# gvanhoy/gr-liquiddsp

Hardware: AMD Instinct MI355X
Metric: Msamples/s through flex_rx (QPSK r1/2 1024B) (higher is better)
Workload: dtype f32; 1 GPU; flex_rx single stream per GPU, 20000000 samples (10 Msym), PSK4 r=1/2 (CONV_V27), 1024-B payload, CRC-24, 256-sample gaps, CFO/phase/delay + AWGN Es/N0=20 dB; frames_decoded_ok=1154, streams_per_gpu=1, blocks_in_flight=12, stage_events=none (fxrx_set_timing level 0), steps=1415, passes=independent captures (reset between passes), segments=256, repairs=0

## Files before the change

### gr-liquiddsp_amd/csrc/fx_host.cpp

```cpp
#include <hip/hip_runtime.h>
#include <algorithm>
#include <chrono>
#include <cmath>
#include <cstdio>
#include <cstdlib>
#include <cstring>
#include <memory>
#include <string>
#include <vector>
#include "../../include/fxrx.h"
#include "fx_device.h"
#include "fx_codec.hpp"
#include "fx_launch.h"
#include "fx_traffic.h"

namespace {

thread_local std::string g_err;
void set_err(const std::string &s) { g_err = s; }

#define HIP_OK(expr)                                                                          \
    do {                                                                                      \
        hipError_t e_ = (expr);                                                               \
        if (e_ != hipSuccess) {                                                               \
// ... 648 lines not shown
    if (!detect && c->cfg.soft_decision && (sl.d_soft.reserve(8 * sl.byte_cap) || (c->cfg.want_framesyms && sl.h_soft.reserve(8 * sl.byte_cap)))) return FXRX_ERR_HIP;
#ifdef FX_STAMPS
    if (!detect && sl.d_pres.reserve(chain_slots)) return FXRX_ERR_HIP;
#endif
    std::memcpy(sl.hp_desc.p, jobs.data(), NJ * sizeof(FxWalkJob));
    uint32_t *hl = reinterpret_cast<uint32_t *>(sl.hp_desc.p + o_list);
    if (!early.empty()) std::memcpy(hl, early.data(), early.size() * sizeof(uint32_t));
    if (!late.empty()) std::memcpy(hl + early.size(), late.data(), late.size() * sizeof(uint32_t));
    if (!spec.empty()) std::memcpy(hl + NJ, spec.data(), spec.size() * sizeof(uint32_t));
    std::memcpy(sl.hp_desc.p + o_streams, sds.data(), NS * sizeof(FxStreamDesc));
    const uint32_t *d_list = sl.job_list();

    const double tp2 = g_prof_on ? prof_now() : 0.0;
    if (!sl.ingest.empty()) {
        std::vector<IngestJob> todo; todo.swap(sl.ingest);
        const size_t bytes = iq_sample_bytes(sl.ingest_fmt);
        for (const IngestJob &j : todo) {
            const void *src = j.dev_src;
            if (!src) { HIP_OK(hipMemcpyAsync(sl.d_raw[j.stream].p, j.host_src, j.n * bytes, hipMemcpyHostToDevice, st)); src = sl.d_raw[j.stream].p; }
            HIP_OK(fx_launch_ingest(st, sl.ingest_fmt, src, sl.d_in[j.stream].p, (size_t)j.n, sl.ingest_scale, (unsigned)c->n_cus));
        }
    }
    HIP_OK(fx_launch_upload(st, sl.hp_desc.p, sl.d_desc.p, desc_bytes, (unsigned)c->n_cus));
    const int tl = c->timing_level >= 0 ? c->timing_level : (c->depth > 1 ? 0 : 2);
    sl.timing_level = tl;
    if (c->debug_walk_twice > 0) HIP_OK(fx_launch_prescan(st, (unsigned)spec.size(), sl.ps_words, sl.jobs(), d_list + NJ, c->d_tables));
    for (int rep = 0; rep < c->debug_walk_twice; rep++) HIP_OK(launch_walk(c, sl, st, d_list, (unsigned)early.size()));
    if (tl >= 2) HIP_OK(hipEventRecord(sl.ev[kEvStart], st));
    if (c->debug_walk_twice <= 0) HIP_OK(fx_launch_prescan(st, (unsigned)spec.size(), sl.ps_words, sl.jobs(), d_list + NJ, c->d_tables));
    HIP_OK(launch_walk(c, sl, st, d_list, (unsigned)early.size()));
    const bool verify = !detect && c->skip_seek && !sl.force_noskip;
    hipStream_t cst = st;
    if (!late.empty()) {
        if (verify) {
            HIP_OK(fx_launch_copy_u32(st, &sl.hdr_walk()->n_runs, &sl.hdr_walk()->runs_done));
            HIP_OK(launch_seekverify(c, sl, st, c->verify_per_cu * (unsigned)c->n_cus, 0u));
        }
        if (!c->st_chain) {
            int lo = 0, hi = 0;
            HIP_OK(hipDeviceGetStreamPriorityRange(&lo, &hi));
            HIP_OK(hipStreamCreateWithPriority(&c->st_chain, hipStreamNonBlocking, hi));
        }
        HIP_OK(hipEventRecord(sl.ev[kEvHandover], st));
        cst = c->st_chain;
        HIP_OK(hipStreamWaitEvent(cst, sl.ev[kEvHandover], 0));
        if (c->prev_chain) HIP_OK(hipStreamWaitEvent(cst, c->prev_chain, 0));
        HIP_OK(launch_walk(c, sl, cst, d_list + early.size(), (unsigned)late.size()));
    }
    if (tl >= 2) HIP_OK(hipEventRecord(sl.ev[kEvWalk], cst));
    if (verify)
        HIP_OK(launch_seekverify(c, sl, cst, late.empty() ? c->verify_per_cu * (unsigned)c->n_cus : (unsigned)std::min<size_t>((size_t)c->verify_per_cu * (size_t)c->n_cus, std::max<size_t>(64, 16 * late.size())), 1u));
    if (tl >= 2) HIP_OK(hipEventRecord(sl.ev[kEvVerify], cst));
    if (late.empty() && c->prev_chain) HIP_OK(hipStreamWaitEvent(cst, c->prev_chain, 0));
    if (c->carry_reader[(b + 1) % 3]) HIP_OK(hipStreamWaitEvent(cst, c->carry_reader[(b + 1) % 3], 0));
    const double tp3 = g_prof_on ? prof_now() : 0.0;
    const int rb = enqueue_back(c, sl, kChainFast, cst, may_defer);
    if (g_prof_on) { const double tp4 = prof_now(); g_prof[1] += tp1 - tp0; g_prof[2] += tp2 - tp1; g_prof[3] += tp3 - tp2; g_prof[4] += tp4 - tp3; g_prof_n++; }
    return rb;
}

static FxVbpreMember vbpre_member(Slot &sl, uint32_t first_wave, uint32_t n_waves)
{
    return FxVbpreMember{ sl.d_pjobs.p, sl.dec_list(kDecBatch), sl.hdr_pay(), sl.d_hard.p, sl.d_bufA.p, sl.d_bufB.p, sl.h_out.p, sl.h_recs.p, sl.h_hdr.p, first_wave, n_waves };
}
static int launch_tails(fxrx_ctx_s *c, Slot *const *m, unsigned n)
{
    hipStream_t st = m[n - 1]->st;
    for (unsigned i = 0; i + 1 < n; i++) HIP_OK(hipStreamWaitEvent(st, m[i]->ev[kEvMf], 0));
    auto done = [&]() -> int {
        for (unsigned i = 0; i < n; i++) { HIP_OK(hipEventRecord(m[i]->ev[kEvDone], st)); m[i]->tail_launched = true; m[i]->tail_st = st; }
        if (n > 1) { c->gang_launches++; c->gang_members += n; }
        return 0;
    };
    {
        FxPllGang g; unsigned waves[FX_GANG_MAX]; g.n = n;
        for (unsigned i = 0; i < n; i++) { const Slot &sl = *m[i]; g.m[i] = FxPllMember{ sl.d_pjobs.p, sl.d_pll_list.p, sl.hdr_pay(), sl.d_symraw.p, sl.d_symraw.p, sl.d_hard.p, sl.h_recs.p }; waves[i] = sl.tail.pll_waves; }
        HIP_OK(fx_launch_paypll(&g, waves, c->pll_waves, st, c->d_tables));
    }
    for (unsigned i = 0; i < n; i++) if (m[i]->timing_level >= 1) HIP_OK(hipEventRecord(m[i]->ev[kEvPll], st));
    if (c->debug_stop_after == 6) return done();
    for (unsigned i = 0; i < n; i++) {
        Slot &sl = *m[i];
        if (c->cfg.soft_decision) {
            HIP_OK(fx_launch_softdemod(sl.tail.mf_grid, st, sl.d_pjobs.p, sl.d_mf_job.p, sl.d_mf_c0.p, sl.hdr_pay(), sl.d_symraw.p, sl.d_hard.p, sl.d_soft.p, c->d_tables));
            if (c->cfg.want_framesyms) HIP_OK(hipMemcpyAsync(sl.h_soft.p, sl.d_soft.p, 8 * sl.byte_cap, hipMemcpyDeviceToHost, st));
        }
        HIP_OK(launch_decoders(c, sl, st, 0u, sl.tail.plain, sl.tail.rs));
    }
    {
        FxVbpreGang g; g.n = n;
        for (unsigned i = 0; i < n; i++) g.m[i] = vbpre_member(*m[i], 0u, m[i]->vb_blk ? m[i]->tail.vb_pre : 0u);
        HIP_OK(fx_launch_vbpre(&g, st, c->d_tables, c->vb_clean ? 1 : 0, c->vb_early_tail && c->vb_clean ? 1 : 0));
    }
    for (unsigned i = 0; i < n; i++) {
        Slot &sl = *m[i];
        if (sl.vb_blk) HIP_OK(launch_trellis(c, sl, st, sl.tail.vb_items, sl.tail.vb_packed, sl.tail.with_fix, sl.tail.vb_fin, sl.tail.fb));
        if (sl.timing_level >= 2) HIP_OK(hipEventRecord(sl.ev[kEvDec], st));
        if (c->cfg.want_framesyms) HIP_OK(fx_launch_symcopy(2u * (unsigned)c->n_cus, st, sl.hdr_pay(), sl.d_symraw.p, sl.h_framesyms.p));
    }
    return done();
}

static int close_gang(fxrx_ctx_s *c)
{
    if (c->gang.empty()) return 0;
    if (c->gang.size() > FX_GANG_MAX) { set_err("open gang larger than FX_GANG_MAX (internal error)"); return FXRX_ERR_STATE; }
    Slot *m[FX_GANG_MAX]; unsigned n = 0;
    for (Slot *s : c->gang) m[n++] = s;
    c->gang.clear();
    return launch_tails(c, m, n);
}

static int enqueue_back(fxrx_ctx_s *c, Slot &sl, int chain_mode, hipStream_t chain_st, bool may_defer)
{
    const unsigned NS = c->cfg.n_streams; const bool detect = c->cfg.mode == FXRX_MODE_DETECTOR;
    const uint64_t b = sl.seq; const uint32_t chain_slots = sl.chain_cap; hipStream_t st = sl.st;
    sl.tail_launched = true; sl.tail_st = st;
    if (chain_mode == kChainFull)
        HIP_OK(fx_launch_chain(detect ? FX_MODE_DETECT : FX_MODE_FLEXRX, c->cfg.equalizer ? 1 : 0, c->cfg.soft_header ? 1 : 0, NS, st, sl.streams(), sl.jobs(), (uint32_t)sl.NJ, sl.d_wres.p, sl.d_frames.p, sl.d_chain.p,
                               sl.d_chain_count.p, sl.d_runs.p, sl.run_cap, sl.hdr_walk(), c->chain_slow ? 1u : 0u, c->d_tables));
    else if (chain_mode == kChainFast) {
        hipStream_t cs = chain_st ? chain_st : st;
        sl.inchain = !c->chain_slow && (c->inchain_repair == 2 || (c->inchain_repair == 1 && c->inchain_left > 0));
        if (c->inchain_left) c->inchain_left--;
        if (!sl.inchain) HIP_OK(launch_chainfast(c, sl, cs, kStitch));
        else {
            HIP_OK(launch_chainfast(c, sl, cs, kStitchPass1));
            HIP_OK(launch_walk(c, sl, cs, sl.d_req.p, (unsigned)std::min<size_t>(2 * sl.NJ, 64), kWalkRequestsInChain));
            HIP_OK(launch_chainfast(c, sl, cs, kStitchPass2));
        }
    }
    HIP_OK(hipEventRecord(sl.ev[kEvChain], chain_mode == kChainFast && chain_st ? chain_st : st));
    if (chain_mode == kChainFast && chain_st && chain_st != st) HIP_OK(hipStreamWaitEvent(st, sl.ev[kEvChain], 0));
    c->prev_chain = sl.ev[kEvChain];
    {
        FxPlanArgs a;
        a.streams = sl.streams(); a.nstreams = NS; a.detect = detect ? 1u : 0u; a.eq = c->cfg.equalizer ? 1u : 0u; a.vb_blk = sl.vb_blk;
        a.chain = sl.d_chain.p; a.chain_count = sl.d_chain_count.p; a.stream_base = sl.d_stream_base.p;
        a.pjobs = sl.d_pjobs.p; a.recs = sl.h_recs.p;
        a.mf_job = sl.d_mf_job.p; a.mf_c0 = sl.d_mf_c0.p; a.mf_cap = sl.mf_cap;
        a.pll_list = sl.d_pll_list.p; a.dec_list = sl.dec_list(kDecPlain); a.list_cap = sl.list_cap();
        a.vb_items = sl.d_vb_items.p; a.vb_cap = sl.vb_cap;
        a.hdr = sl.hdr_walk(); a.hdr_pay = sl.hdr_pay(); a.hdr_host = sl.h_hdr.p; a.ws = sl.d_plan_ws.p;
        HIP_OK(fx_launch_plan(st, c->plan_grid ? c->plan_grid : (unsigned)std::min<uint64_t>(64, c->traffic.frames / 2048 + 1), c->plan_fused ? 1 : 0, c->plan_threads, a));
    }
    const int tl = sl.timing_level;
    if (tl >= 2) HIP_OK(hipEventRecord(sl.ev[kEvPlan], st));
    if (c->debug_stop_after == 4) { c->carry_reader[b % 3] = nullptr; HIP_OK(hipEventRecord(sl.ev[kEvDone], st)); return 0; }
    if (!detect) {
        const TailPlan plan = plan_tail(c->traffic, TailCaps{ chain_slots, sl.mf_cap, sl.vb_cap, sl.vb_blk }, TailKnobs{ c->depth, c->n_cus, c->mf_per_cu, c->vb_debug, c->vb_early_tail, c->vb_clean });
        HIP_OK(fx_launch_paymf(plan.mf_grid, c->cfg.equalizer ? 1 : 0, st, sl.d_pjobs.p, sl.d_mf_job.p, sl.d_mf_c0.p, sl.hdr_pay(), sl.d_chain.p, sl.d_symraw.p, c->d_tables));
        HIP_OK(hipEventRecord(sl.ev[kEvMf], st));
        c->carry_reader[b % 3] = sl.ev[kEvMf];
        if (c->debug_stop_after == 5) { HIP_OK(hipEventRecord(sl.ev[kEvDone], st)); return 0; }
        sl.tail = plan;
        if (sl.vb_blk && c->traffic.trellis_left) c->traffic.trellis_left--;
        sl.timing.trellis_launched = plan.vb_fin ? 1 : 0;
        unsigned ahead = 0;
        for (unsigned k = 0; k < c->inflight; k++) ahead += c->slots[(c->tail + k) % (c->depth + 1)]->tail_launched ? 1u : 0u;
        const unsigned G = c->tail_gang;
        if (G >= 2 && may_defer && c->depth >= 4 && c->traffic.seen && !c->debug_stop_after && tl <= 1 && ahead >= G) {
            sl.tail_launched = false; sl.tail_st = nullptr;
            c->gang.push_back(&sl);
            return c->gang.size() >= G ? close_gang(c) : 0;
        }
        { const int r = close_gang(c); if (r) return r; }
        Slot *one = &sl;
        return launch_tails(c, &one, 1u);
    } else {
        if (c->cfg.want_framesyms) HIP_OK(launch_detwin(c, sl, 0u, sl.win_reserved, false));
        HIP_OK(hipEventRecord(sl.ev[kEvMf], st));
        if (tl >= 1) HIP_OK(hipEventRecord(sl.ev[kEvPll], st));
        if (tl >= 2) HIP_OK(hipEventRecord(sl.ev[kEvDec], st));
        c->carry_reader[b % 3] = sl.ev[kEvMf];
    }
    HIP_OK(hipEventRecord(sl.ev[kEvDone], st));
    return 0;
}

static int prepare_ingest(fxrx_ctx_s *c, Slot &sl, const void *const *iq, const uint64_t *n_samples, int on_device, int fmt)
{
    const unsigned NS = c->cfg.n_streams;
    const size_t bytes = iq_sample_bytes(fmt);
    sl.ingest.clear();
    for (unsigned s = 0; s < NS; s++)
        if (n_samples[s] && (!iq[s] || (reinterpret_cast<uintptr_t>(iq[s]) & (bytes - 1)))) {
            set_err("fxrx_submit_fmt: integer IQ must be aligned to its sample size (sc16: 4 bytes, sc8: 2 bytes)"); return FXRX_ERR_ARG;
        }
    if (sl.d_in.size() < NS) sl.d_in.resize(NS);
    if (sl.d_raw.size() < NS) sl.d_raw.resize(NS);
    std::vector<IngestJob> jobs;
    for (unsigned s = 0; s < NS; s++) {
        const uint64_t nn = n_samples[s];
        if (sl.d_in[s].reserve(nn + 1)) return FXRX_ERR_HIP;
        if (!nn) continue;
        IngestJob j; j.stream = s; j.n = nn;
        if (on_device) j.dev_src = iq[s];
        else if (!(nn * bytes <= c->ingest_kernel_max && pinned_device_ptr(iq[s], &j.dev_src, 0u))) {
            j.dev_src = nullptr; j.host_src = iq[s];
            if (sl.d_raw[s].reserve(nn * bytes + 16)) return FXRX_ERR_HIP;
        }
        jobs.push_back(j);
    }
    sl.ingest.swap(jobs); sl.ingest_fmt = fmt; sl.ingest_scale = c->iq_scale[fmt];
    return 0;
}

static int submit_block(fxrx_ctx *c, const void *const *iq, const uint64_t *n_samples, int on_device, int fmt)
{
    if (!c || !iq || !n_samples) { set_err("fxrx_submit: null argument"); return FXRX_ERR_ARG; }
    if (iq_sample_bytes(fmt) == 0) { set_err("fxrx_submit_fmt: unknown IQ format"); return FXRX_ERR_ARG; }
    if (c->inflight >= c->depth) { set_err("fxrx_submit: pipeline full, call fxrx_collect first"); return FXRX_ERR_STATE; }
    HIP_OK(hipSetDevice(c->cfg.device));
    const auto t_enter = std::chrono::steady_clock::now();
    const unsigned NS = c->cfg.n_streams;
    const unsigned nslots = c->depth + 1;
    Slot &sl = *c->slots[c->head];
    sl.ingest.clear();
    if (fmt != FXRX_IQ_FC32) { const int r = prepare_ingest(c, sl, iq, n_samples, on_device, fmt); if (r) return r; }
    sl.out.clear(); sl.timing = fxrx_timing{};
    sl.kept_hops = sl.kept_cheap = sl.kept_vhops = sl.kept_vfail = sl.kept_repairs = 0;
    const unsigned noskip_before = c->noskip_left;
    sl.force_noskip = c->noskip_left > 0; if (c->noskip_left) c->noskip_left--;
    sl.seq = c->seq;
    sl.x.assign(NS, nullptr); sl.n.assign(n_samples, n_samples + NS); sl.snap.assign(NS, StreamSnap{});
    if (sl.d_in.size() < NS) sl.d_in.resize(NS);
    struct Undo { fxrx_ctx_s *c; std::vector<StreamState> st; unsigned noskip; bool armed = true;
                  ~Undo() { if (armed) { c->st = st; c->noskip_left = noskip; } } } undo{ c, c->st, noskip_before };
    uint64_t total_new = 0;
    for (unsigned s = 0; s < NS; s++) {
        StreamState &S = c->st[s];
        const uint64_t nn = n_samples[s];
        total_new += nn;
        if (fmt != FXRX_IQ_FC32) sl.x[s] = sl.d_in[s].p;
// ... 513 lines not shown
```

### gr-liquiddsp_amd/csrc/fx_kernels.hip

```cpp
#include <hip/hip_runtime.h>
#include <algorithm>
#include "fx_device.h"
#include "fx_launch.h"
#include "fx_vbclean.h"
#include "fx_rsgmd.h"

#define HALF         256

template <int WW> struct WalkLdsT {
    static constexpr int WAVES = WW;
    static constexpr bool SWEEP_PAIRS = WW == 4;
    float2 win[FX_NFFT];
    float2 X[FX_NFFT];
    float2 S[FX_NFFT];
    float2 scr[WW][576];
    float2 v[640];
    float2 P[256];
    float  m2[FX_NFFT];
    float2 hdr[FX_HDR_SYM];
    float2 cw[(WW + 1) * FX_HOP + 8];
    __device__ __forceinline__ float2 *scr2(int wave) { return wave < 2 ? v + 576 * wave : cw + 576 * (wave - 2); }
    float2 pb[16];
    float2 eqw[16];
    float  taps[FX_MF_TAPS];
// ... 2177 lines not shown
                const uint32_t g = t0 + k, sub = tid & 15u;
                for (uint32_t b = sub; b < kp.y; b += 16u) if (kp.x + b < a.vb_cap) { a.vb_items[kp.x + b] = g; a.vb_items[a.vb_cap + kp.x + b] = b; }
                for (uint32_t c = sub; c < kp.w; c += 16u) if (kp.z + c < a.mf_cap) { a.mf_job[kp.z + c] = g; a.mf_c0[kp.z + c] = c * 1024u; }
            }
            __syncthreads();
        }
    }
    plan_pad_lists<NT>(cnt, sh.cls_base, sh.vbc_base, a);
    PLAN_TICK(st6_);
    __threadfence(); __syncthreads();
    PLAN_TICK(st7_);
    if (tid == 0) {
#ifdef FX_STAMPS
        sh.h.stamp[1] = st1_; sh.h.stamp[2] = st2_; sh.h.stamp[6] = st6_; sh.h.stamp[7] = st7_;
#endif
        plan_fill_hdr(sh.h, N, run, cnt, sh.cls_base, sh.vbc_base, a);
    }
    __syncthreads();
    plan_mirror_hdr<NT>(sh.h, a);
}

extern "C" hipError_t fx_launch_plan(hipStream_t st, unsigned grid, int fused, unsigned threads, const FxPlanArgs &a)
{
    const unsigned g = grid < 1u ? 1u : (grid > PLAN_MAXG ? PLAN_MAXG : grid);
    if (fused && g == 1u) {
        if (threads == 512u) hipLaunchKernelGGL((fx_planfused_kernel<512>), dim3(1), dim3(512), 0, st, a);
        else if (threads == 256u) hipLaunchKernelGGL((fx_planfused_kernel<256>), dim3(1), dim3(256), 0, st, a);
        else return hipErrorInvalidValue;
    } else {
        hipLaunchKernelGGL(fx_plan_kernel, dim3(g), dim3(PLAN_THREADS), 0, st, a);
        hipLaunchKernelGGL(fx_planlists_kernel, dim3(g), dim3(PLAN_THREADS), 0, st, a);
    }
    return hipGetLastError();
}
extern "C" unsigned fx_plan_ws_words(void) { return PW_WORDS; }

#define PMF_THREADS 256
#define PMF_SYMS    1024
#define PMF_SPAN    (2 * PMF_SYMS + FX_MF_TAPS)

__global__ __launch_bounds__(PMF_THREADS)
void fx_paymf_kernel(const FxPayJob *jobs, const uint32_t *blk_job, const uint32_t *blk_c0, const FxBlockHdr *hdr, const FxFrame *chain, float2 *sym_raw,
                     const FxTables *T)
{
    constexpr int LEAD = FX_EQ_TAPS - 1;
    __shared__ float2 v[PMF_SPAN + LEAD + 4];
    __shared__ float2 u[2 * PMF_SYMS + FX_EQ_TAPS];
    __shared__ float2 eqw[16];
    __shared__ float taps[FX_MF_TAPS];
    const uint32_t nitems = hdr->n_mfblk;
    const int tid = threadIdx.x;
    const float2 *sc = T->sc;
    for (uint32_t bi = blockIdx.x; bi < nitems; bi += gridDim.x) {
        const FxPayJob job = jobs[blk_job[bi]];
        const uint32_t c0 = blk_c0[bi];
        const uint32_t ns = min((uint32_t)PMF_SYMS, job.nsym - c0);
        const int64_t sym0 = (int64_t)FX_SYM0_PAY + FX_EQ_DELAY;
        const int64_t nlo = sym_sample(sym0 + c0, job.mfc0) - LEAD - (FX_MF_TAPS - 1);
        const int64_t nhi = sym_sample(sym0 + c0 + ns - 1, job.mfc0);
        const int span = (int)(nhi - nlo + 1);
        const XSrc xs = make_xsrc(job.x, job.xa_end, 0);
        __syncthreads();
        if (tid < FX_MF_TAPS) taps[tid] = T->proto[job.pfb + FX_NPFB * tid];
        if (tid < 16) eqw[tid] = tid < FX_EQ_TAPS ? chain[job.chain_idx].eq[tid] : make_float2(0.0f, 0.0f);
        for (int m = tid; m < span; m += PMF_THREADS) {
            const int64_t nn = nlo + m;
            v[m] = derot(xld(xs, job.start + nn), job.mix_th + job.mix_dl * (uint32_t)nn, sc);
        }
        __syncthreads();
        const int nu = span - (FX_MF_TAPS - 1);
        for (int m = tid; m < nu; m += PMF_THREADS) {
            const float2 y = mf_sum<7>(v, taps, m + (FX_MF_TAPS - 1));
            u[m] = make_float2(y.x * job.mf_scale, y.y * job.mf_scale);
        }
        __syncthreads();
        for (uint32_t i = tid; i < ns; i += PMF_THREADS) {
            const int nc = (int)(sym_sample(sym0 + c0 + i, job.mfc0) - nlo) - (FX_MF_TAPS - 1);
            sym_raw[(size_t)job.sym_off + c0 + i] = eq_sum16(u + nc - (FX_EQ_TAPS - 1), eqw);
        }
    }
}

#define PMF4_STRIDE 274
extern "C" __global__ __launch_bounds__(PMF_THREADS)
void fx_paymf4_kernel(const FxPayJob *jobs, const uint32_t *blk_job, const uint32_t *blk_c0, const FxBlockHdr *hdr, float2 *sym_raw, const FxTables *T)
{
    __shared__ float2 ph[8 * PMF4_STRIDE];
    __shared__ __attribute__((aligned(16))) float taps[FX_MF_TAPS];
    static_assert(FX_MF_TAPS == 28 && PMF_SYMS == 4 * PMF_THREADS, "tile below: 28 taps, four symbols per thread");
    static_assert(PMF4_STRIDE >= (PMF_SPAN + 8) / 8 + 5, "phase arrays hold the span plus the slack phantom symbols read");
    const uint32_t nitems = hdr->n_mfblk;
    const int tid = threadIdx.x;
    const float2 *sc = T->sc;
    for (uint32_t bi = blockIdx.x; bi < nitems; bi += gridDim.x) {
        const FxPayJob job = jobs[blk_job[bi]];
        const uint32_t c0 = blk_c0[bi];
        const uint32_t ns = min((uint32_t)PMF_SYMS, job.nsym - c0);
        const int64_t nlo = sym_sample((int64_t)FX_SYM0_PAY + c0, job.mfc0) - (FX_MF_TAPS - 1);
        const int span = 2 * (int)ns + (FX_MF_TAPS - 2);
        const float2 *px = job.x, *pa = job.xa_end;
        const int64_t p0 = job.start + nlo;
        const uint32_t th0 = job.mix_th + job.mix_dl * (uint32_t)nlo, dl = job.mix_dl;
        __syncthreads();
        if (tid < FX_MF_TAPS) taps[tid] = T->proto[job.pfb + FX_NPFB * tid];
        constexpr int NLD = (PMF_SPAN + PMF_THREADS - 1) / PMF_THREADS;
        float2 raw[NLD];
#pragma unroll
        for (int k = 0; k < NLD; k++) {
            const int m = tid + PMF_THREADS * k;
            const int64_t p = p0 + m;
            raw[k] = m < span ? (p < 0 ? pa[p] : px[p]) : make_float2(0.0f, 0.0f);
        }
#pragma unroll
        for (int k = 0; k < NLD; k++) {
            const int m = tid + PMF_THREADS * k;
            const int j = m >> 1;
            if (m < span) ph[((m & 1) * 4 + (j & 3)) * PMF4_STRIDE + (j >> 2)] = derot(raw[k], th0 + dl * (uint32_t)m, sc);
        }
        __syncthreads();
        if (4u * (uint32_t)tid < ns) {
            float2 e[17], o[17];
#pragma unroll
            for (int j = 0; j < 17; j++) {
                e[j] = ph[(j & 3) * PMF4_STRIDE + tid + (j >> 2)];
                o[j] = ph[(4 + (j & 3)) * PMF4_STRIDE + tid + (j >> 2)];
            }
            float h[FX_MF_TAPS];
#pragma unroll
            for (int q = 0; q < FX_MF_TAPS / 4; q++) { const float4 t4 = reinterpret_cast<const float4 *>(taps)[q]; h[4 * q] = t4.x; h[4 * q + 1] = t4.y; h[4 * q + 2] = t4.z; h[4 * q + 3] = t4.w; }
            float yr[4], yi[4];
#pragma unroll
            for (int r = 0; r < 4; r++) {
                float ar = 0.0f, ai = 0.0f;
#pragma unroll
                for (int k = 0; k < 14; k++) {
                    ar = fmaf(h[2 * k], o[13 + r - k].x, ar); ai = fmaf(h[2 * k], o[13 + r - k].y, ai);
                    ar = fmaf(h[2 * k + 1], e[13 + r - k].x, ar); ai = fmaf(h[2 * k + 1], e[13 + r - k].y, ai);
                }
                yr[r] = ar * job.mf_scale; yi[r] = ai * job.mf_scale;
            }
            float4 *dst = reinterpret_cast<float4 *>(sym_raw + (size_t)job.sym_off + c0 + 4u * (uint32_t)tid);
            dst[0] = make_float4(yr[0], yi[0], yr[1], yi[1]);
            dst[1] = make_float4(yr[2], yi[2], yr[3], yi[3]);
        }
    }
}

extern "C" hipError_t fx_launch_paymf(unsigned grid, int eq, hipStream_t st, const FxPayJob *jobs, const uint32_t *blk_job, const uint32_t *blk_c0, const FxBlockHdr *hdr,
                                      const FxFrame *chain, float2 *sym_raw, const FxTables *T)
{
    if (grid == 0) return hipSuccess;
    if (eq) hipLaunchKernelGGL(fx_paymf_kernel, dim3(grid), dim3(PMF_THREADS), 0, st, jobs, blk_job, blk_c0, hdr, chain, sym_raw, T);
    else hipLaunchKernelGGL(fx_paymf4_kernel, dim3(grid), dim3(PMF_THREADS), 0, st, jobs, blk_job, blk_c0, hdr, sym_raw, T);
    return hipGetLastError();
}

#define PLL_THREADS 64
#define PLL_MAX_WAVES 4
#define PLL_BLK     8

__device__ __forceinline__ void pll_load8(const float4 *p, float4 b[4]) { b[0] = p[0]; b[1] = p[1]; b[2] = p[2]; b[3] = p[3]; }

template <int MS>
__device__ __forceinline__ unsigned pll_demod(float2 r, unsigned &prev, const float2 *sc, float2 &xh, float &pe)
{
    if constexpr (MS == FX_MODEM_PSK2 || MS == FX_MODEM_PSK4) {
        unsigned idx; float pr, pim;
        if constexpr (MS == FX_MODEM_PSK2) {
            const bool neg = !(r.x > 0.0f);
            idx = neg ? 1u : 0u;
            xh = make_float2(neg ? -1.0f : 1.0f, 0.0f);
            pr = neg ? -r.x : r.x; pim = neg ? -r.y : r.y;
        } else {
            const bool horiz = fabsf(r.x) >= fabsf(r.y);
            const bool neg = horiz ? !(r.x > 0.0f) : !(r.y > 0.0f);
            idx = (horiz ? 0u : 1u) + (neg ? 2u : 0u);
            const float sg = neg ? -1.0f : 1.0f;
            xh = horiz ? make_float2(sg, 0.0f) : make_float2(0.0f, sg);
            const float a = horiz ? r.x : r.y, b = horiz ? r.y : -r.x;
            pr = neg ? -a : a; pim = neg ? -b : b;
        }
        (void)pr;
        pe = pim;
        return gray_enc(idx);
    } else {
        return modem_demod((unsigned)MS, modem_bps((unsigned)MS), r, prev, sc, xh, pe);
    }
}

template <int MS, bool TAIL>
__device__ __forceinline__ void pll_block8(const float4 (&cur)[4], unsigned live, uint32_t &th, float &fq, float &evm, unsigned &prev, const float2 *sc,
                                           float4 *out, uint2 *hd)
{
    float rr[2 * PLL_BLK]; unsigned h0 = 0, h1 = 0;
    float wc, ws; sincos_u32(th, sc, wc, ws);
#pragma unroll
    for (int k = 0; k < PLL_BLK; k++) {
        const float4 v4 = cur[k >> 1];
        const float2 y = (k & 1) ? make_float2(v4.z, v4.w) : make_float2(v4.x, v4.y);
        float2 r = make_float2(fmaf(y.x, wc, y.y * ws), fmaf(y.y, wc, -(y.x * ws))), xh; float pe;
        unsigned pv = prev;
        const unsigned s = pll_demod<MS>(r, pv, sc, xh, pe);
        if (!TAIL || (unsigned)k < live) {
            float dr = r.x - xh.x, di = r.y - xh.y;
            evm += fmaf(dr, dr, di * di);
            fq = fmaf(pe, 68356.5248f, fq);
            const float t = phase_step(fmaf(pe, 6835652.5f, fq));
            th += (uint32_t)(int)t;
            float cd, sd; sincos_small(t, cd, sd);
            const float c2 = fmaf(wc, cd, -(ws * sd)), s2 = fmaf(ws, cd, wc * sd);
            wc = c2; ws = s2;
            prev = pv;
        }
        rr[2 * k] = r.x; rr[2 * k + 1] = r.y;
        if (k < 4) h0 |= s << (8 * k); else h1 |= s << (8 * (k - 4));
    }
#pragma unroll
    for (int k = 0; k < 4; k++) out[k] = make_float4(rr[4 * k], rr[4 * k + 1], rr[4 * k + 2], rr[4 * k + 3]);
    *hd = make_uint2(h0, h1);
}

template <int MS>
__device__ __forceinline__ void pll_frame(uint32_t f, const FxPayJob *jobs, const float2 *sc, const float2 *sym_raw, float2 *framesyms, uint8_t *hard, FxOutRec *recs)
{
    if (f == 0xFFFFFFFFu) return;
    const FxPayJob job = jobs[f];
    const float4 *in = reinterpret_cast<const float4 *>(sym_raw + job.sym_off);
// ... 2165 lines not shown
```

### gr-liquiddsp_amd/csrc/fx_traffic.h

```cpp
#pragma once
#include <algorithm>
#include <stdint.h>
#include "fx_common.h"

constexpr unsigned kTrellisHold = 8;
constexpr uint32_t kFallbackWaves = 32;

struct Traffic {
    bool seen = false;
    uint64_t samples = 0, frames = 0;
    uint64_t plain = 0, rs = 0;
    uint64_t batch = 0, vb_items = 0;
    uint64_t vb_steps = 0;
    uint64_t vb_fix = 0;
    uint64_t fb = 0;
    uint64_t mf_items = 0;
    uint32_t verify_per = 4;
    unsigned trellis_left = 0;

    void observe(const FxBlockHdr &h, uint64_t vb_rep, uint64_t vb_clean, bool vb_early, uint64_t n_samples, int n_cus)
    {
        samples = n_samples; frames = h.n_frames; plain = h.n_dec_plain; batch = h.n_dec_batch; vb_items = h.n_vb_items; mf_items = h.n_mfblk;
        vb_steps = (uint64_t)h.vb_want * (h.vb_blk ? h.vb_blk : 1u);
        fb = h.n_vb_fallback; vb_fix = h.n_vb_fallback + vb_rep;
        if (vb_early && h.n_dec_batch > vb_clean) trellis_left = kTrellisHold;
        rs = h.n_dec_rs ? h.n_dec_rs : rs - std::min<uint64_t>(rs, std::max<uint64_t>(1, rs / 8));
        if (h.verify_hops) verify_per = (uint32_t)std::min<uint64_t>(16, std::max<uint64_t>(1, ((uint64_t)h.verify_hops + 4ull * n_cus - 1) / (4ull * n_cus)));
        seen = true;
    }
};

inline uint32_t with_margin(uint64_t count, uint64_t cap, uint64_t extra = 64, uint64_t floor = 0) { return (uint32_t)std::min(cap, std::max(floor, count + count / 2 + extra)); }

struct TailPlan {
    uint32_t pll_waves = 0, mf_grid = 0;
    uint32_t plain = 0, rs = 0;
    uint32_t vb_pre = 0, vb_items = 0, vb_fin = 0, fb = 0;
    int vb_packed = 0, with_fix = 0;
    bool vb_early = false;
};
struct TailCaps { uint32_t chain_slots, mf_cap, vb_cap, vb_blk; };
struct TailKnobs { unsigned depth; int n_cus; uint32_t mf_per_cu, vb_debug; bool vb_early_tail, vb_clean; };

inline TailPlan plan_tail(const Traffic &t, const TailCaps &cap, const TailKnobs &k)
{
    const uint64_t slots = cap.chain_slots, cus = (uint64_t)k.n_cus;
    TailPlan p;
    p.pll_waves = (t.frames ? with_margin(t.frames, slots) : cap.chain_slots) / 64 + FX_PLL_CLASSES;
    p.mf_grid = (uint32_t)std::min<uint64_t>(cap.mf_cap, k.mf_per_cu ? k.mf_per_cu * cus : std::max<uint64_t>(8 * cus, t.mf_items + t.mf_items / 8 + 64));
    p.vb_early = cap.vb_blk && k.vb_early_tail && k.vb_clean;
    const bool trellis = cap.vb_blk && (!p.vb_early || !t.seen || k.vb_debug || t.trellis_left > 0);
    if (!t.seen) {
        p.plain = cap.chain_slots; p.rs = std::min<uint32_t>(cap.chain_slots, 64u);
        if (cap.vb_blk) { p.vb_pre = p.fb = cap.chain_slots; p.vb_items = cap.vb_cap; }
    } else {
        p.plain = t.plain || !cap.vb_blk ? with_margin(t.plain, slots) : 0u;
        p.rs = t.rs ? with_margin(t.rs, slots) : 0u;
        if (cap.vb_blk) {
            p.vb_pre = with_margin(t.batch, slots);
            p.vb_items = trellis ? with_margin(t.vb_items, cap.vb_cap, 1024) : 0u;
            p.fb = trellis && (t.fb || k.vb_debug) ? with_margin(t.fb, slots, 16, kFallbackWaves) : 0u;
        }
    }
    p.vb_fin = trellis ? p.vb_pre : 0u;
    if (cap.vb_blk) {
        p.vb_packed = (k.depth > 1 || t.vb_items > 64ull * 4ull * cus * 3ull / 2ull) ? 1 : 0;
        p.with_fix = (!t.seen || t.vb_fix || k.vb_debug) ? 1 : 0;
    }
    return p;
}

struct LateWork {
    bool more_plain = false;
    bool more_rs = false;
    bool more_batch_frames = false;
    bool more_batch_items = false;
    bool more_fb = false;
    bool late_trellis = false;
    bool more_batch() const { return more_batch_frames || more_batch_items; }
    bool any() const { return more_plain || more_rs || more_batch() || more_fb || late_trellis; }
    void count(uint64_t n[6]) const { n[0] += more_plain; n[1] += more_rs; n[2] += more_batch_frames; n[3] += more_batch_items; n[4] += more_fb; n[5] += late_trellis; }
};

inline LateWork late_work(const TailPlan &p, const FxBlockHdr &h, uint32_t vb_blk)
{
    LateWork w;
    const bool no_trellis = vb_blk && p.vb_fin == 0;
    w.more_plain = h.n_dec_plain > p.plain; w.more_rs = h.n_dec_rs > 0 && p.rs == 0;
    w.more_batch_frames = h.n_dec_batch > p.vb_pre; w.more_batch_items = !no_trellis && h.n_vb_items > p.vb_items;
    w.more_fb = vb_blk && h.n_vb_fallback > p.fb;
    w.late_trellis = no_trellis && !w.more_batch() && h.vb_dirty != 0u;
    return w;
}
```

Before: 41140 Msamples/s.

## Software-pipeline payload matched filter with double-buffered LDS and persistent grid

The payload matched-filter kernel becomes a persistent loop over work items with double-buffered shared-memory phase arrays, so the global loads for the next block are issued while the current block is filtered. It adds a 16-byte vectorized load path for aligned contiguous spans, reads the taps into scalar registers via readfirstlane, and replaces __syncthreads with an explicit LDS fence and barrier. The non-equalizer launch grid shrinks to a fixed four blocks per CU instead of scaling with item count, and soft-demod keeps the old grid sizing. The larger register and LDS footprint may reduce occupancy, and a small fixed grid may leave CUs idle on short bursts.

```diff
diff --git a/gr-liquiddsp_amd/csrc/fx_host.cpp b/gr-liquiddsp_amd/csrc/fx_host.cpp
--- a/gr-liquiddsp_amd/csrc/fx_host.cpp
+++ b/gr-liquiddsp_amd/csrc/fx_host.cpp
@@ -754,7 +754,7 @@
     for (unsigned i = 0; i < n; i++) {
         Slot &sl = *m[i];
         if (c->cfg.soft_decision) {
-            HIP_OK(fx_launch_softdemod(sl.tail.mf_grid, st, sl.d_pjobs.p, sl.d_mf_job.p, sl.d_mf_c0.p, sl.hdr_pay(), sl.d_symraw.p, sl.d_hard.p, sl.d_soft.p, c->d_tables));
+            HIP_OK(fx_launch_softdemod(sl.tail.sd_grid, st, sl.d_pjobs.p, sl.d_mf_job.p, sl.d_mf_c0.p, sl.hdr_pay(), sl.d_symraw.p, sl.d_hard.p, sl.d_soft.p, c->d_tables));
             if (c->cfg.want_framesyms) HIP_OK(hipMemcpyAsync(sl.h_soft.p, sl.d_soft.p, 8 * sl.byte_cap, hipMemcpyDeviceToHost, st));
         }
         HIP_OK(launch_decoders(c, sl, st, 0u, sl.tail.plain, sl.tail.rs));
@@ -821,7 +821,7 @@
     if (c->debug_stop_after == 4) { c->carry_reader[b % 3] = nullptr; HIP_OK(hipEventRecord(sl.ev[kEvDone], st)); return 0; }
     if (!detect) {
         const TailPlan plan = plan_tail(c->traffic, TailCaps{ chain_slots, sl.mf_cap, sl.vb_cap, sl.vb_blk }, TailKnobs{ c->depth, c->n_cus, c->mf_per_cu, c->vb_debug, c->vb_early_tail, c->vb_clean });
-        HIP_OK(fx_launch_paymf(plan.mf_grid, c->cfg.equalizer ? 1 : 0, st, sl.d_pjobs.p, sl.d_mf_job.p, sl.d_mf_c0.p, sl.hdr_pay(), sl.d_chain.p, sl.d_symraw.p, c->d_tables));
+        HIP_OK(fx_launch_paymf(c->cfg.equalizer ? plan.sd_grid : plan.mf_grid, c->cfg.equalizer ? 1 : 0, st, sl.d_pjobs.p, sl.d_mf_job.p, sl.d_mf_c0.p, sl.hdr_pay(), sl.d_chain.p, sl.d_symraw.p, c->d_tables));
         HIP_OK(hipEventRecord(sl.ev[kEvMf], st));
         c->carry_reader[b % 3] = sl.ev[kEvMf];
         if (c->debug_stop_after == 5) { HIP_OK(hipEventRecord(sl.ev[kEvDone], st)); return 0; }
diff --git a/gr-liquiddsp_amd/csrc/fx_kernels.hip b/gr-liquiddsp_amd/csrc/fx_kernels.hip
--- a/gr-liquiddsp_amd/csrc/fx_kernels.hip
+++ b/gr-liquiddsp_amd/csrc/fx_kernels.hip
@@ -2283,43 +2283,119 @@
 }
 
 #define PMF4_STRIDE 274
-extern "C" __global__ __launch_bounds__(PMF_THREADS)
-void fx_paymf4_kernel(const FxPayJob *jobs, const uint32_t *blk_job, const uint32_t *blk_c0, const FxBlockHdr *hdr, float2 *sym_raw, const FxTables *T)
-{
-    __shared__ float2 ph[8 * PMF4_STRIDE];
-    __shared__ __attribute__((aligned(16))) float taps[FX_MF_TAPS];
+#define PMF4_NWIDE  (PMF_SYMS / PMF_THREADS)
+struct Pmf4Item {
+    const float2 *px, *pa;
+    int64_t p0;
+    uint32_t th0, dl, ns, pfb;
+    float scale;
+    size_t out;
+};
+FX_DEV Pmf4Item pmf4_item(const FxPayJob *__restrict__ jobs, uint32_t ji, uint32_t c0)
+{
+    const FxPayJob &job = jobs[ji];
+    Pmf4Item it;
+    const int64_t nlo = sym_sample((int64_t)FX_SYM0_PAY + c0, job.mfc0) - (FX_MF_TAPS - 1);
+    it.px = job.x; it.pa = job.xa_end;
+    it.p0 = job.start + nlo;
+    it.dl = job.mix_dl; it.th0 = job.mix_th + job.mix_dl * (uint32_t)nlo;
+    it.ns = min((uint32_t)PMF_SYMS, job.nsym - c0);
+    it.pfb = job.pfb; it.scale = job.mf_scale;
+    it.out = (size_t)job.sym_off + c0;
+    return it;
+}
+FX_DEV bool pmf4_wide(const Pmf4Item &it)
+{
+    const int span = 2 * (int)it.ns + (FX_MF_TAPS - 2);
+    const bool in_x = it.p0 >= 0, in_a = it.p0 + span <= 0;
+    const float2 *b = (in_x ? it.px : it.pa) + it.p0;
+    return (in_x || in_a) && (reinterpret_cast<uintptr_t>(b) & 15u) == 0;
+}
+typedef float Pmf4V2 __attribute__((ext_vector_type(2)));
+typedef float Pmf4V4 __attribute__((ext_vector_type(4)));
+typedef const Pmf4V2 __attribute__((address_space(1))) *Pmf4Src;
+typedef const Pmf4V4 __attribute__((address_space(1))) *Pmf4Src4;
+FX_DEV float2 pmf4_ld2(Pmf4Src p) { const Pmf4V2 q = *p; return make_float2(q.x, q.y); }
+FX_DEV float4 pmf4_ld4(Pmf4Src p) { const Pmf4V4 q = *(Pmf4Src4)p; return make_float4(q.x, q.y, q.z, q.w); }
+FX_DEV void pmf4_load(const Pmf4Item &it, bool wide, int tid, float4 (&rw)[PMF4_NWIDE], float2 &rt)
+{
+    const int span = 2 * (int)it.ns + (FX_MF_TAPS - 2);
+    const Pmf4Src px = (Pmf4Src)it.px, pa = (Pmf4Src)it.pa;
+    const int64_t p0 = it.p0;
+    if (wide) {
+        const Pmf4Src b = (p0 >= 0 ? px : pa) + p0;
+#pragma unroll
+        for (int k = 0; k < PMF4_NWIDE; k++) rw[k] = pmf4_ld4(b + min(2 * (tid + PMF_THREADS * k), span - 2));
+        rt = pmf4_ld2(b + min(2 * PMF_SYMS + tid, span - 1));
+    } else {
+#pragma unroll
+        for (int k = 0; k < 2 * PMF4_NWIDE + 1; k++) {
+            const int64_t p = p0 + min(tid + PMF_THREADS * k, span - 1);
+            const float2 v = pmf4_ld2((p < 0 ? pa : px) + p);
+            if (k == 2 * PMF4_NWIDE) rt = v;
+            else if (k & 1) { rw[k >> 1].z = v.x; rw[k >> 1].w = v.y; }
+            else { rw[k >> 1].x = v.x; rw[k >> 1].y = v.y; }
+        }
+    }
+}
+FX_DEV void pmf4_stage(float2 *ph, const Pmf4Item &it, bool wide, int tid, const float4 (&rw)[PMF4_NWIDE], float2 rt, const float2 *sc)
+{
+    const int span = 2 * (int)it.ns + (FX_MF_TAPS - 2);
+    constexpr int N = 2 * PMF4_NWIDE + 1;
+    int m[N]; float2 v[N];
+#pragma unroll
+    for (int k = 0; k < PMF4_NWIDE; k++) {
+        m[2 * k] = wide ? 2 * (tid + PMF_THREADS * k) : tid + PMF_THREADS * 2 * k;
+        m[2 * k + 1] = wide ? m[2 * k] + 1 : m[2 * k] + PMF_THREADS;
+        v[2 * k] = make_float2(rw[k].x, rw[k].y); v[2 * k + 1] = make_float2(rw[k].z, rw[k].w);
+    }
+    m[N - 1] = 2 * PMF_SYMS + tid; v[N - 1] = rt;
+#pragma unroll
+    for (int k = 0; k < N; k++) v[k] = derot(v[k], it.th0 + it.dl * (uint32_t)m[k], sc);
+#pragma unroll
+    for (int k = 0; k < N; k++) {
+        const int j = m[k] >> 1;
+        if (m[k] < span) ph[((m[k] & 1) * 4 + (j & 3)) * PMF4_STRIDE + (j >> 2)] = v[k];
+    }
+}
+
+extern "C" __global__ __launch_bounds__(PMF_THREADS, 4)
+void fx_paymf4_kernel(const FxPayJob *__restrict__ jobs, const uint32_t *__restrict__ blk_job, const uint32_t *__restrict__ blk_c0, const FxBlockHdr *__restrict__ hdr,
+                      float2 *__restrict__ sym_raw, const FxTables *__restrict__ T)
+{
+    __shared__ float2 ph2[2][8 * PMF4_STRIDE];
+    __shared__ __attribute__((aligned(16))) float taps2[2][FX_MF_TAPS];
     static_assert(FX_MF_TAPS == 28 && PMF_SYMS == 4 * PMF_THREADS, "tile below: 28 taps, four symbols per thread");
     static_assert(PMF4_STRIDE >= (PMF_SPAN + 8) / 8 + 5, "phase arrays hold the span plus the slack phantom symbols read");
-    const uint32_t nitems = hdr->n_mfblk;
+    static_assert(PMF_SPAN <= (2 * PMF4_NWIDE + 1) * PMF_THREADS, "nine samples per thread cover the span");
+    const uint64_t nitems = hdr->n_mfblk, step = gridDim.x;
     const int tid = threadIdx.x;
     const float2 *sc = T->sc;
-    for (uint32_t bi = blockIdx.x; bi < nitems; bi += gridDim.x) {
-        const FxPayJob job = jobs[blk_job[bi]];
-        const uint32_t c0 = blk_c0[bi];
-        const uint32_t ns = min((uint32_t)PMF_SYMS, job.nsym - c0);
-        const int64_t nlo = sym_sample((int64_t)FX_SYM0_PAY + c0, job.mfc0) - (FX_MF_TAPS - 1);
-        const int span = 2 * (int)ns + (FX_MF_TAPS - 2);
-        const float2 *px = job.x, *pa = job.xa_end;
-        const int64_t p0 = job.start + nlo;
-        const uint32_t th0 = job.mix_th + job.mix_dl * (uint32_t)nlo, dl = job.mix_dl;
-        __syncthreads();
-        if (tid < FX_MF_TAPS) taps[tid] = T->proto[job.pfb + FX_NPFB * tid];
-        constexpr int NLD = (PMF_SPAN + PMF_THREADS - 1) / PMF_THREADS;
-        float2 raw[NLD];
-#pragma unroll
-        for (int k = 0; k < NLD; k++) {
-            const int m = tid + PMF_THREADS * k;
-            const int64_t p = p0 + m;
-            raw[k] = m < span ? (p < 0 ? pa[p] : px[p]) : make_float2(0.0f, 0.0f);
-        }
-#pragma unroll
-        for (int k = 0; k < NLD; k++) {
-            const int m = tid + PMF_THREADS * k;
-            const int j = m >> 1;
-            if (m < span) ph[((m & 1) * 4 + (j & 3)) * PMF4_STRIDE + (j >> 2)] = derot(raw[k], th0 + dl * (uint32_t)m, sc);
-        }
-        __syncthreads();
-        if (4u * (uint32_t)tid < ns) {
+    uint64_t bi = blockIdx.x;
+    if (bi >= nitems) return;
+    Pmf4Item cur = pmf4_item(jobs, blk_job[bi], blk_c0[bi]), nxt = cur;
+    bool cur_wide = pmf4_wide(cur), nxt_wide = false;
+    float4 rw[PMF4_NWIDE]; float2 rt;
+    const int tap = min(tid, FX_MF_TAPS - 1);
+    float tapv = T->proto[cur.pfb + FX_NPFB * tap];
+    pmf4_load(cur, cur_wide, tid, rw, rt);
+    bool has1 = bi + step < nitems, has2 = has1 && bi + 2 * step < nitems;
+    if (has1) nxt = pmf4_item(jobs, blk_job[bi + step], blk_c0[bi + step]);
+    uint32_t ji2 = has2 ? blk_job[bi + 2 * step] : 0u, c02 = has2 ? blk_c0[bi + 2 * step] : 0u;
+    for (int set = 0; ; set ^= 1) {
+        float2 *ph = ph2[set];
+        float *taps = taps2[set];
+        if (tid < FX_MF_TAPS) taps[tid] = tapv;
+        pmf4_stage(ph, cur, cur_wide, tid, rw, rt, sc);
+        if (has1) { nxt_wide = pmf4_wide(nxt); tapv = T->proto[nxt.pfb + FX_NPFB * tap]; pmf4_load(nxt, nxt_wide, tid, rw, rt); }
+        Pmf4Item nn = nxt;
+        if (has2) nn = pmf4_item(jobs, ji2, c02);
+        const bool has3 = has2 && bi + 3 * step < nitems;
+        if (has3) { ji2 = blk_job[bi + 3 * step]; c02 = blk_c0[bi + 3 * step]; }
+        __builtin_amdgcn_fence(__ATOMIC_RELEASE, "workgroup", "local");
+        __builtin_amdgcn_s_barrier();
+        __builtin_amdgcn_fence(__ATOMIC_ACQUIRE, "workgroup", "local");
+        if (4u * (uint32_t)tid < cur.ns) {
             float2 e[17], o[17];
 #pragma unroll
             for (int j = 0; j < 17; j++) {
@@ -2329,6 +2405,8 @@
             float h[FX_MF_TAPS];
 #pragma unroll
             for (int q = 0; q < FX_MF_TAPS / 4; q++) { const float4 t4 = reinterpret_cast<const float4 *>(taps)[q]; h[4 * q] = t4.x; h[4 * q + 1] = t4.y; h[4 * q + 2] = t4.z; h[4 * q + 3] = t4.w; }
+#pragma unroll
+            for (int q = 0; q < FX_MF_TAPS; q++) h[q] = __int_as_float(__builtin_amdgcn_readfirstlane(__float_as_int(h[q])));
             float yr[4], yi[4];
 #pragma unroll
             for (int r = 0; r < 4; r++) {
@@ -2338,12 +2416,14 @@
                     ar = fmaf(h[2 * k], o[13 + r - k].x, ar); ai = fmaf(h[2 * k], o[13 + r - k].y, ai);
                     ar = fmaf(h[2 * k + 1], e[13 + r - k].x, ar); ai = fmaf(h[2 * k + 1], e[13 + r - k].y, ai);
                 }
-                yr[r] = ar * job.mf_scale; yi[r] = ai * job.mf_scale;
+                yr[r] = ar * cur.scale; yi[r] = ai * cur.scale;
             }
-            float4 *dst = reinterpret_cast<float4 *>(sym_raw + (size_t)job.sym_off + c0 + 4u * (uint32_t)tid);
+            float4 *dst = reinterpret_cast<float4 *>(sym_raw + cur.out + 4u * (uint32_t)tid);
             dst[0] = make_float4(yr[0], yi[0], yr[1], yi[1]);
             dst[1] = make_float4(yr[2], yi[2], yr[3], yi[3]);
         }
+        if (!has1) break;
+        cur = nxt; cur_wide = nxt_wide; nxt = nn; has1 = has2; has2 = has3; bi += step;
     }
 }
 
diff --git a/gr-liquiddsp_amd/csrc/fx_traffic.h b/gr-liquiddsp_amd/csrc/fx_traffic.h
--- a/gr-liquiddsp_amd/csrc/fx_traffic.h
+++ b/gr-liquiddsp_amd/csrc/fx_traffic.h
@@ -4,6 +4,7 @@
 #include "fx_common.h"
 
 constexpr unsigned kTrellisHold = 8;
+constexpr uint32_t kMfPerCu = 4;
 constexpr uint32_t kFallbackWaves = 32;
 
 struct Traffic {
@@ -34,6 +35,7 @@
 
 struct TailPlan {
     uint32_t pll_waves = 0, mf_grid = 0;
+    uint32_t sd_grid = 0;
     uint32_t plain = 0, rs = 0;
     uint32_t vb_pre = 0, vb_items = 0, vb_fin = 0, fb = 0;
     int vb_packed = 0, with_fix = 0;
@@ -47,7 +49,8 @@
     const uint64_t slots = cap.chain_slots, cus = (uint64_t)k.n_cus;
     TailPlan p;
     p.pll_waves = (t.frames ? with_margin(t.frames, slots) : cap.chain_slots) / 64 + FX_PLL_CLASSES;
-    p.mf_grid = (uint32_t)std::min<uint64_t>(cap.mf_cap, k.mf_per_cu ? k.mf_per_cu * cus : std::max<uint64_t>(8 * cus, t.mf_items + t.mf_items / 8 + 64));
+    p.sd_grid = (uint32_t)std::min<uint64_t>(cap.mf_cap, k.mf_per_cu ? k.mf_per_cu * cus : std::max<uint64_t>(8 * cus, t.mf_items + t.mf_items / 8 + 64));
+    p.mf_grid = (uint32_t)std::max<uint64_t>(1, std::min<uint64_t>(cap.mf_cap, (k.mf_per_cu ? k.mf_per_cu : kMfPerCu) * cus));
     p.vb_early = cap.vb_blk && k.vb_early_tail && k.vb_clean;
     const bool trellis = cap.vb_blk && (!p.vb_early || !t.seen || k.vb_debug || t.trellis_left > 0);
     if (!t.seen) {
```

Result: no change. 40840 Msamples/s (-0.7%).
